# vr308/Generalised-Gaussian-Processes

Hardware: AMD Instinct MI355X
Metric: ELBO evals/sec (higher is better)
Workload: dtype f64

## Files before the change

generalised-gaussian-processes_amd/csrc/sgp_suffstats_fwd.hip:

```cpp
#include "sgp_common.hpp"
#include "sgp_stream.hpp"
#include "sgp_dense.hpp"
#include "sgp_composite.hpp"
#include "sgp_ctx.hpp"
#include <cstdlib>

namespace sgp {

static_assert(TIMING_SLOTS == CTX_TIMING_SLOTS, "timing slots");
size_t stream_kfu_budget() { return cur_ctx().kfu_budget; }

void timing_begin(int slot, hipStream_t st) {
  Ctx& c = cur_ctx();
  if (!c.timing) return;
  if (!c.ev_ready) {
    bool ok = true;
    for (int s = 0; s < TIMING_SLOTS; ++s)
      for (int k = 0; k < 2; ++k) ok = (hipEventCreate(&c.ev[s][k]) == hipSuccess) && ok;
    if (!ok) return;
    c.ev_ready = 1;
  }
  if (hipEventRecord(c.ev[slot][0], st) != hipSuccess) c.ev_used[slot] = 0;
}
void timing_end(int slot, hipStream_t st) {
// ... 236 lines not shown
        }
      };
#define SGP_DUMMY(cc, st) dummy(cc, st)
#else
#define SGP_DUMMY(cc, st)
#endif
      for (; c + 1 < c1; c += 2) {
        if (c + 2 < c1) fetch(c + 2, stA);
        mfma_chunk(0);
        SGP_DUMMY(c + 1, stB);
        stash(1, stB);
        __syncthreads();
        if (c + 3 < c1) fetch(c + 3, stB);
        mfma_chunk(1);
        if (c + 2 < c1) { SGP_DUMMY(c + 2, stA); }
        if (c + 2 < c1) stash(0, stA);
        __syncthreads();
      }
#ifdef SGP_AB_DIAG_DUMMY_ASM
      if (sink == 1.2345e300) out[0] = sink;
#endif
      if (c < c1) mfma_chunk(0);
    }
  
}

  if constexpr (BALANCED) {
    switch (wave) {
      case 0: diag_store<0>(acc, out, accumulate, l15, l4); break;
      case 1: diag_store<1>(acc, out, accumulate, l15, l4); break;
      case 2: diag_store<2>(acc, out, accumulate, l15, l4); break;
      default: diag_store<3>(acc, out, accumulate, l15, l4); break;
    }
    return;
  }
  {
#pragma unroll
    for (int u = 0; u < 4; ++u)
#pragma unroll
      for (int v = 0; v < VB; ++v)
#pragma unroll
        for (int r = 0; r < 4; ++r) {
          const int row = wi * 64 + u * 16 + l4 + 4 * r;
          const int col = wj * WCOLS + v * 16 + l15;
          double* dst = out + row * TILE + col;
          *dst = accumulate ? *dst + acc[u][v][r] : acc[u][v][r];
        }
  }
}

template <int NW, bool GLDS, bool SKIP>
__global__ __launch_bounds__(NW * 64, NW / 2) void syrk_tile_kernel(const double* __restrict__ Kfu, int Mp, int64_t nchunks,
                                                                    SplitMap smap, int ntiles, int accumulate,
                                                                    double* __restrict__ slab, int nsplit) {
  __shared__ double Ks[2][NB][KROW];
  const int id = blockIdx.x;
  const int xcd = id & 7;
  const int jj = id >> 3;
  const int full = (nsplit >> 3) * ntiles;
  int t, split;
  if (jj < full) {
    t = jj % ntiles;
    split = (jj / ntiles) * 8 + xcd;
  } else {
    const int rem = (nsplit & 7) * ntiles, per = (rem + 7) >> 3;
    const int u = xcd * per + (jj - full);
    if (jj - full >= per || u >= rem) return;
    t = u % ntiles;
    split = (nsplit & ~7) + u / ntiles;
  }
  int ti = (int)((sqrt(8.0 * t + 1.0) - 1.0) * 0.5);
  while ((ti + 1) * (ti + 2) / 2 <= t) ++ti;
  while (ti * (ti + 1) / 2 > t) --ti;
  const int tj = t - ti * (ti + 1) / 2;
  int64_t c0, c1;
  split_range(smap, split, nchunks, c0, c1);
  double* out = slab + ((size_t)split * ntiles + t) * (TILE * TILE);
  if (ti == tj)
    syrk_tile<true, NW, GLDS, SKIP>(Ks, Kfu, Mp, c0, c1, ti * TILE, tj * TILE, accumulate, out);
  else
    syrk_tile<false, NW, GLDS, SKIP>(Ks, Kfu, Mp, c0, c1, ti * TILE, tj * TILE, accumulate, out);
}

__global__ __launch_bounds__(256) void reduce_phi_kernel(const double* __restrict__ slab, int nsplit, int ntiles,
                                                         int M, double scale, double* __restrict__ Phi) {
  __shared__ double tile[32][33];
  const int t = blockIdx.x;
  int bi = (int)((sqrt(8.0 * t + 1.0) - 1.0) * 0.5);
  while ((bi + 1) * (bi + 2) / 2 <= t) ++bi;
  while (bi * (bi + 1) / 2 > t) --bi;
  const int bj = t - bi * (bi + 1) / 2;
  const int tx = threadIdx.x & 31, ty = threadIdx.x >> 5;
  const int Ti = (bi * 32) / TILE, Tj = (bj * 32) / TILE;
  const int tileidx = Ti * (Ti + 1) / 2 + Tj;
  const double* base = slab + (size_t)tileidx * (TILE * TILE);
  const size_t sstride = (size_t)ntiles * (TILE * TILE);
#pragma unroll
  for (int k = 0; k < 4; ++k) {
    const int lr = ty + 8 * k;
    const int gi = bi * 32 + lr, gj = bj * 32 + tx;
    double s = 0.0;
    if (gi >= gj) {
      const size_t off = (size_t)(gi - Ti * TILE) * TILE + (gj - Tj * TILE);
#pragma unroll 8
      for (int sp = 0; sp < nsplit; ++sp) s += base[sp * sstride + off];
    }
    tile[lr][tx] = s * scale;
  }
  __syncthreads();
#pragma unroll
  for (int k = 0; k < 4; ++k) {
    const int lr = ty + 8 * k;
    const int gi = bi * 32 + lr, gj = bj * 32 + tx;
    if (gi < M && gj < M && gi >= gj) Phi[(size_t)gi * M + gj] = tile[lr][tx];
    const int mi = bj * 32 + lr, mj = bi * 32 + tx;
    if (mi < M && mj < M && mj > mi) Phi[(size_t)mi * M + mj] = tile[tx][lr];
  }
}

__global__ __launch_bounds__(256) void bpart_stage1_kernel(const double* __restrict__ bpart, int64_t nrb, int Mp, int G,
                                                           double* __restrict__ tmp) {
  __shared__ double part[4][64];
  const int col = blockIdx.x * 64 + (threadIdx.x & 63), w = threadIdx.x >> 6, g = blockIdx.y;
  double s = 0.0;
  for (int64_t rb = g + (int64_t)w * G; rb < nrb; rb += 4 * (int64_t)G) s += bpart[rb * Mp + col];
  part[w][threadIdx.x & 63] = s;
  __syncthreads();
  if (w == 0) {
    const int l = threadIdx.x;
    tmp[(size_t)g * Mp + col] = (part[0][l] + part[1][l]) + (part[2][l] + part[3][l]);
  }
}

__global__ __launch_bounds__(256) void finalize_stats_kernel(const double* __restrict__ btmp, int G, int Mp, int M,
                                                             const double* __restrict__ yypart, int nyy, double sf2,
                                                             double kappa_val, double* __restrict__ b,
                                                             double* __restrict__ yy, double* __restrict__ kappa) {
  const int m = blockIdx.x * 256 + threadIdx.x;
  if (m < M) {
    double s = 0.0;
#pragma unroll 8
    for (int g = 0; g < G; ++g) s += btmp[(size_t)g * Mp + m];
    b[m] = s * sf2;
  }
  if (blockIdx.x == 0) {
    __shared__ double red[4];
    double s = 0.0;
    for (int i = threadIdx.x; i < nyy; i += 256) s += yypart[i];
    s = block_sum256(s, red);
    if (threadIdx.x == 0) {
      *yy = s;
      *kappa = kappa_val;
    }
  }
}

template <int DP, int ROWS>
static void launch_assemble_rows(int kid, dim3 grid, hipStream_t st, const double* Xs, const double* ys, const double* Zs,
                                 int64_t row0, int64_t N, int M, int Mp, double* Kfu, double* bpart) {
  switch (kid) {
    case SGP_KERNEL_RBF: kfu_assemble_kernel<DP, SGP_KERNEL_RBF, ROWS><<<grid, 256, 0, st>>>(Xs, ys, Zs, row0, N, M, Mp, Kfu, bpart); break;
    case SGP_KERNEL_MATERN32: kfu_assemble_kernel<DP, SGP_KERNEL_MATERN32, ROWS><<<grid, 256, 0, st>>>(Xs, ys, Zs, row0, N, M, Mp, Kfu, bpart); break;
    default: kfu_assemble_kernel<DP, SGP_KERNEL_MATERN52, ROWS><<<grid, 256, 0, st>>>(Xs, ys, Zs, row0, N, M, Mp, Kfu, bpart); break;
  }
}
template <int DP>
static void launch_assemble(int kid, int sub, dim3 grid, hipStream_t st, const double* Xs, const double* ys, const double* Zs,
                            int64_t row0, int64_t N, int M, int Mp, double* Kfu, double* bpart) {
  if (sub == 16) launch_assemble_rows<DP, ASM_ROWS / 16>(kid, grid, st, Xs, ys, Zs, row0, N, M, Mp, Kfu, bpart);
  else if (sub == 8) launch_assemble_rows<DP, ASM_ROWS / 8>(kid, grid, st, Xs, ys, Zs, row0, N, M, Mp, Kfu, bpart);
  else if (sub == 4) launch_assemble_rows<DP, ASM_ROWS / 4>(kid, grid, st, Xs, ys, Zs, row0, N, M, Mp, Kfu, bpart);
  else launch_assemble_rows<DP, ASM_ROWS>(kid, grid, st, Xs, ys, Zs, row0, N, M, Mp, Kfu, bpart);
}

void stream_assemble(const StreamPlan& p, int kid, const double* Xs, const double* ys, const double* Zs, int64_t row0,
                     int64_t rows, int64_t N, int M, double* Kfu, double* bpart, hipStream_t st) {
  dim3 grid((unsigned)(rows / ASM_ROWS * p.asm_sub), (p.Mp + 255) / 256);
  switch (p.DP) {
    case 2: launch_assemble<2>(kid, p.asm_sub, grid, st, Xs, ys, Zs, row0, N, M, p.Mp, Kfu, bpart); break;
    case 4: launch_assemble<4>(kid, p.asm_sub, grid, st, Xs, ys, Zs, row0, N, M, p.Mp, Kfu, bpart); break;
    case 8: launch_assemble<8>(kid, p.asm_sub, grid, st, Xs, ys, Zs, row0, N, M, p.Mp, Kfu, bpart); break;
    case 16: launch_assemble<16>(kid, p.asm_sub, grid, st, Xs, ys, Zs, row0, N, M, p.Mp, Kfu, bpart); break;
    case 24: launch_assemble<24>(kid, p.asm_sub, grid, st, Xs, ys, Zs, row0, N, M, p.Mp, Kfu, bpart); break;
    default: launch_assemble<32>(kid, p.asm_sub, grid, st, Xs, ys, Zs, row0, N, M, p.Mp, Kfu, bpart); break;
  }
}

void stream_prologue(const StreamPlan& p, const KernArgs& ka, const double* X, int64_t ldx, const double* y,
                     const double* Z, int64_t ldz, int64_t N, int M, double* Xs, double* ys, double* Zs, double* yypart,
                     hipStream_t st, const PadSymJob& pad) {
  int gx = 0;
  if (N > 0) {
    const int64_t tot = p.Npad * p.DP;
    gx = (int)((tot + 255) / 256 < 4096 ? (tot + 255) / 256 : 4096);
  }
  const int gz = (p.Mp * p.DP + 255) / 256;
  int gp = 0;
  if (pad.P) {
    const int64_t blocks = ((int64_t)p.Mp * p.Mp + 255) / 256;
// ... 390 lines not shown
  if (Kfu_out) p.sc_rows = p.Npad;
  FwdWs w = carve_fwd(ws, p, Kfu_out == nullptr, qrows);
  if (!ws || ws_bytes < w.bytes) return SGP_ERR_WORKSPACE;
  hipStream_t st = (hipStream_t)stream;

  KernArgs ka;
  for (int j = 0; j < SGP_MAX_DIM; ++j) ka.inv_ls[j] = j < d ? inv_ls[j] : 0.0;
  ka.sf2 = sf2;
  ka.d = d;

  stream_prologue(p, ka, X, ldx, y, Z, ldz, N, M, w.Xs, w.ys, w.Zs, w.yypart, st);
  double* Kfu = Kfu_out ? Kfu_out : w.Kfu;
  const int grid = p.ntiles * p.nsplit;
  if (p.Npad == 0) {
    syrk_tile_kernel<4, false, false><<<grid, 256, 0, st>>>(Kfu, p.Mp, 0, SplitMap{{0, 0, 0, 0}, 1}, p.ntiles, 0, w.slab, p.nsplit);
  }
  auto contract = [&](const double* K, int64_t nchunks, const SplitMap& smap, int nsplit, int accum, double* slab) {
    launch_syrk(cx, K, p.Mp, nchunks, smap, p.ntiles, nsplit, accum, slab, st);
  };
  int nslabs = p.nsplit;
  int head_ns = 0;
  int64_t head_chunks = 0;
  const bool use_i8 = i8_rule(cx.contraction, p.Npad, p.Mp);
  cx.contraction_used = use_i8 ? 1 : 0;
  if (!use_i8) gate = nullptr;
  if (p.Npad > 0 && !use_i8) head_block(p, p.Npad / NB, &head_ns, &head_chunks);
  if (use_i8) {
    const int ns = i8_nsplit(qrows, p.Mp);
    for (int64_t r0 = 0; r0 < p.Npad; r0 += qrows) {
      const int64_t rows = (p.Npad - r0) < qrows ? (p.Npad - r0) : qrows;
      timing_begin(TIMING_ASSEMBLE, st);
      i8_assemble(p, kernel_id, w.Xs, w.ys, w.Zs, r0, rows, N, M, w.Q, Kfu_out ? Kfu_out + (size_t)r0 * p.Mp : nullptr, w.bpart, st);
      timing_end(TIMING_ASSEMBLE, st);
      if (gate && hipStreamWaitEvent(st, gate, 0) != hipSuccess) return SGP_ERR_LAUNCH;
      gate = nullptr;
      timing_begin(TIMING_SYRK, st);
      if (i8_contract(w.Q, p.Mp, rows, ns, r0 > 0 ? 1 : 0, w.slab, st) != SGP_OK) return SGP_ERR_LAUNCH;
      timing_end(TIMING_SYRK, st);
      cx.syrk_timed_rows = rows;
    }
    nslabs = ns;
  } else if (head_ns > 0) {
    const int64_t hrows = head_chunks * NB, trows = p.Npad - hrows, tchunks = trows / NB;
    const bool side = cx.asm_overlap == 1 && side_stream_ready(cx);
    double* head_slab = w.slab + (size_t)p.nsplit * p.ntiles * TILE * TILE;
    const int hcps = (int)((head_chunks + head_ns - 1) / head_ns);
    const int tcps = (int)((tchunks + p.nsplit - 1) / p.nsplit);
    const SplitMap hmap{{0, 0, 0, 0}, hcps < 1 ? 1 : hcps};
    const SplitMap tmap{{p.taper[0], p.taper[1], p.taper[2], p.taper[3]}, tcps < 1 ? 1 : tcps};
    timing_begin(TIMING_ASSEMBLE, st);
    stream_assemble(p, kernel_id, w.Xs, w.ys, w.Zs, 0, hrows, N, M, Kfu, w.bpart, st);
    bool forked = false;
    if (side && hipEventRecord(cx.ev_fork, st) == hipSuccess && hipStreamWaitEvent(cx.side, cx.ev_fork, 0) == hipSuccess) {
      stream_assemble(p, kernel_id, w.Xs, w.ys, w.Zs, hrows, trows, N, M, Kfu + (size_t)hrows * p.Mp, w.bpart, cx.side);
      forked = hipEventRecord(cx.ev_join, cx.side) == hipSuccess;
      if (!forked) (void)hipStreamSynchronize(cx.side);
    } else {
      stream_assemble(p, kernel_id, w.Xs, w.ys, w.Zs, hrows, trows, N, M, Kfu + (size_t)hrows * p.Mp, w.bpart, st);
    }
    timing_end(TIMING_ASSEMBLE, st);
    contract(Kfu, head_chunks, hmap, head_ns, 0, head_slab);
    if (forked && hipStreamWaitEvent(st, cx.ev_join, 0) != hipSuccess) (void)hipStreamSynchronize(cx.side);
    timing_begin(TIMING_SYRK, st);
    contract(Kfu + (size_t)hrows * p.Mp, tchunks, tmap, p.nsplit, 0, w.slab);
    timing_end(TIMING_SYRK, st);
    cx.syrk_timed_rows = trows;
    nslabs = p.nsplit + head_ns;
  } else {
    for (int64_t r0 = 0; r0 < p.Npad; r0 += p.sc_rows) {
      const int64_t rows = (p.Npad - r0) < p.sc_rows ? (p.Npad - r0) : p.sc_rows;
      timing_begin(TIMING_ASSEMBLE, st);
      stream_assemble(p, kernel_id, w.Xs, w.ys, w.Zs, r0, rows, N, M, Kfu, w.bpart, st);
      timing_end(TIMING_ASSEMBLE, st);
      const int64_t nchunks = rows / NB;
      const int cps = (int)((nchunks + p.nsplit - 1) / p.nsplit);
      const SplitMap smap{{p.taper[0], p.taper[1], p.taper[2], p.taper[3]}, cps < 1 ? 1 : cps};
      timing_begin(TIMING_SYRK, st);
      contract(Kfu, nchunks, smap, p.nsplit, r0 > 0 ? 1 : 0, w.slab);
      timing_end(TIMING_SYRK, st);
      cx.syrk_timed_rows = rows;
    }
  }
  const int nb32 = p.Mp / 32;
  reduce_phi_kernel<<<nb32 * (nb32 + 1) / 2, 256, 0, st>>>(w.slab, nslabs, p.ntiles, M, sf2 * sf2, Phi);
  bpart_stage1_kernel<<<dim3(p.Mp / 64, BRED_G), 256, 0, st>>>(w.bpart, p.Npad / ASM_ROWS * (use_i8 ? 1 : p.asm_sub), p.Mp, BRED_G, w.btmp);
  finalize_stats_kernel<<<(M + 255) / 256, 256, 0, st>>>(w.btmp, BRED_G, p.Mp, M, w.yypart, 256, sf2,
                                                         sf2 * (double)N, b, yy, kappa);
  return check_launch();
}

extern "C" size_t sgp_suffstats_whitened_rows_workspace_bytes(int64_t N, int M, int d, int caller_owns_t) {
  if (N < 0 || M <= 0 || d <= 0 || d > SGP_MAX_DIM || M > SGP_MAX_INDUCING) return 0;
  StreamPlan p = make_stream_plan(N, M, d);
  if (caller_owns_t) p.sc_rows = p.Npad;
  return carve_wh_rows(nullptr, p, caller_owns_t != 0).bytes;
}
extern "C" int sgp_suffstats_fwd_whitened_rows(const double* X, int64_t ldx, const double* y, const double* Z, int64_t ldz,
                                               const double* inv_ls, double sf2, int64_t N, int M, int d, int kernel_id,
                                               const double* kuu_linv, double* W, double* u, double* yy, double* kappa, double* T_out,
                                               void* ws, size_t ws_bytes, sgp_stream_t stream) {
  Ctx& cx = cur_ctx();
  if (!Z || !inv_ls || !kuu_linv || !W || !u || !yy || !kappa || N < 0 || M <= 0 || d <= 0 || ldz < d) return SGP_ERR_ARG;
  if (N > 0 && (!X || !y || ldx < d)) return SGP_ERR_ARG;
  if (kernel_id < 0 || kernel_id >= SGP_KERNEL_COMPOSITE) return SGP_ERR_ARG;
  if (d > SGP_MAX_DIM || M > SGP_MAX_INDUCING) return SGP_ERR_DIM;
  StreamPlan p = make_stream_plan(N, M, d);
  if (T_out) p.sc_rows = p.Npad;
  WhRowsWs w = carve_wh_rows(ws, p, T_out != nullptr);
  if (!ws || ws_bytes < w.bytes) return SGP_ERR_WORKSPACE;
  hipStream_t st = (hipStream_t)stream;
  KernArgs ka;
  for (int j = 0; j < SGP_MAX_DIM; ++j) ka.inv_ls[j] = j < d ? inv_ls[j] : 0.0;
  ka.sf2 = sf2;
  ka.d = d;
  stream_prologue(p, ka, X, ldx, y, Z, ldz, N, M, w.f.Xs, w.f.ys, w.f.Zs, w.f.yypart, st);
  transpose_square(kuu_linv, p.Mp, w.R, st);
  if (p.Npad == 0)
    syrk_tile_kernel<4, false, false><<<p.ntiles * p.nsplit, 256, 0, st>>>(w.f.Kfu, p.Mp, 0, SplitMap{{0, 0, 0, 0}, 1}, p.ntiles, 0, w.f.slab,
                                                                           p.nsplit);
  for (int64_t r0 = 0; r0 < p.Npad; r0 += p.sc_rows) {
    const int64_t rows = (p.Npad - r0) < p.sc_rows ? (p.Npad - r0) : p.sc_rows;
    double* T = T_out ? T_out + (size_t)r0 * p.Mp : w.T;
    timing_begin(TIMING_ASSEMBLE, st);
    stream_assemble(p, kernel_id, w.f.Xs, w.f.ys, w.f.Zs, r0, rows, N, M, w.f.Kfu, w.f.bpart, st);
    timing_end(TIMING_ASSEMBLE, st);
    GemmDesc g;
    g.A = w.f.Kfu; g.lda = p.Mp; g.B = w.R; g.ldb = p.Mp; g.C = T; g.ldc = p.Mp;
    g.m = (int)rows; g.n = p.Mp; g.k = p.Mp; g.khi_mask = 2;
    gemm(g, st);
    tpart_kernel<<<dim3((unsigned)(rows / ASM_ROWS), (p.Mp + 255) / 256), 256, 0, st>>>(T, w.f.ys, r0, p.Mp, w.f.bpart);
    const int64_t nchunks = rows / NB;
    const int cps = (int)((nchunks + p.nsplit - 1) / p.nsplit);
    const SplitMap smap{{p.taper[0], p.taper[1], p.taper[2], p.taper[3]}, cps < 1 ? 1 : cps};
    timing_begin(TIMING_SYRK, st);
    launch_syrk(cx, T, p.Mp, nchunks, smap, p.ntiles, p.nsplit, r0 > 0 ? 1 : 0, w.f.slab, st);
    timing_end(TIMING_SYRK, st);
    cx.syrk_timed_rows = rows;
  }
  const int nb32 = p.Mp / 32;
  reduce_phi_kernel<<<nb32 * (nb32 + 1) / 2, 256, 0, st>>>(w.f.slab, p.nsplit, p.ntiles, M, sf2 * sf2, W);
  bpart_stage1_kernel<<<dim3(p.Mp / 64, BRED_G), 256, 0, st>>>(w.f.bpart, p.Npad / ASM_ROWS, p.Mp, BRED_G, w.f.btmp);
  finalize_stats_kernel<<<(M + 255) / 256, 256, 0, st>>>(w.f.btmp, BRED_G, p.Mp, M, w.f.yypart, 256, sf2, sf2 * (double)N, u, yy, kappa);
  return check_launch();
}


extern "C" size_t sgp_suffstats_extended_workspace_bytes(int64_t N, int M, int d) {
  if (N < 0 || M <= 0 || d <= 0 || d > SGP_MAX_DIM || M > SGP_MAX_INDUCING) return 0;
  StreamPlan p = make_stream_plan(N, M, d);
  return carve_ext(nullptr, p, p.sc_rows).bytes;
}
extern "C" int sgp_suffstats_fwd_extended(const double* X, int64_t ldx, const double* y, const double* Z, int64_t ldz,
                                          const double* inv_ls, double sf2, int64_t N, int M, int d, int kernel_id,
                                          const double* kuu_linv, int level, double* W, double* u, double* yy, double* kappa,
                                          double* Kfu_out, void* ws, size_t ws_bytes, sgp_stream_t stream) {
  return sgp_suffstats_fwd_extended_ex(X, ldx, y, Z, ldz, inv_ls, sf2, N, M, d, kernel_id, kuu_linv, level, W, u, yy, kappa, Kfu_out,
                                       nullptr, ws, ws_bytes, stream);
}
extern "C" int sgp_suffstats_fwd_extended_ex(const double* X, int64_t ldx, const double* y, const double* Z, int64_t ldz,
                                             const double* inv_ls, double sf2, int64_t N, int M, int d, int kernel_id,
                                             const double* kuu_linv, int level, double* W, double* u, double* yy, double* kappa,
                                             double* Kfu_out, double* phi_diag, void* ws, size_t ws_bytes, sgp_stream_t stream) {
  return sgp_suffstats_fwd_extended_f16(X, ldx, y, Z, ldz, inv_ls, sf2, N, M, d, kernel_id, kuu_linv, level, W, u, yy, kappa, Kfu_out, nullptr,
                                        phi_diag, ws, ws_bytes, stream);
}
extern "C" int sgp_suffstats_fwd_extended_f16(const double* X, int64_t ldx, const double* y, const double* Z, int64_t ldz,
                                              const double* inv_ls, double sf2, int64_t N, int M, int d, int kernel_id,
                                              const double* kuu_linv, int level, double* W, double* u, double* yy, double* kappa,
                                              double* Kfu_out, uint16_t* Kfu_f16_out, double* phi_diag, void* ws, size_t ws_bytes,
                                              sgp_stream_t stream) {
  if (Kfu_f16_out && !Kfu_out) return SGP_ERR_ARG;
  if (!Z || !inv_ls || !kuu_linv || !W || !u || !yy || !kappa || N < 0 || M <= 0 || d <= 0 || ldz < d) return SGP_ERR_ARG;
  if (N > 0 && (!X || !y || ldx < d)) return SGP_ERR_ARG;
  if (kernel_id < 0 || kernel_id >= SGP_KERNEL_COMPOSITE || level < 1 || level > 2) return SGP_ERR_ARG;
  if (d > SGP_MAX_DIM || M > SGP_MAX_INDUCING) return SGP_ERR_DIM;
  StreamPlan p = make_stream_plan(N, M, d);
  const int64_t qrows = p.sc_rows;
  ExtWs w = carve_ext(ws, p, qrows);
  if (!ws || ws_bytes < w.bytes) return SGP_ERR_WORKSPACE;
  hipStream_t st = (hipStream_t)stream;
  KernArgs ka;
  for (int j = 0; j < SGP_MAX_DIM; ++j) ka.inv_ls[j] = j < d ? inv_ls[j] : 0.0;
  ka.sf2 = sf2;
  ka.d = d;
  stream_prologue(p, ka, X, ldx, y, Z, ldz, N, M, w.Xs, w.ys, w.Zs, w.yypart, st);
  const int ns = i8_nsplit(qrows > 0 ? qrows : 1, p.Mp);
  const size_t nslab = (size_t)ns * p.ntiles * TILE * TILE;
  if (p.Npad == 0) {
    fill_zero(w.slab, nslab, st);
    fill_zero(w.slab_lo, nslab, st);
  }
  for (int64_t r0 = 0; r0 < p.Npad; r0 += qrows) {
    const int64_t rows = (p.Npad - r0) < qrows ? (p.Npad - r0) : qrows;
    timing_begin(TIMING_ASSEMBLE, st);
    i8_assemble(p, kernel_id, w.Xs, w.ys, w.Zs, r0, rows, N, M, w.Q, Kfu_out ? Kfu_out + (size_t)r0 * p.Mp : nullptr, w.bpart, st,
                Kfu_f16_out ? Kfu_f16_out + (size_t)r0 * p.Mp : nullptr);
    timing_end(TIMING_ASSEMBLE, st);
    timing_begin(TIMING_SYRK, st);
    if (i8_contract(w.Q, p.Mp, rows, ns, r0 > 0 ? 1 : 0, w.slab, st, w.slab_lo, level) != SGP_OK) return SGP_ERR_LAUNCH;
    timing_end(TIMING_SYRK, st);
  }
  const int nb32 = p.Mp / 32;
  reduce_phi_dd_kernel<<<nb32 * (nb32 + 1) / 2, 256, 0, st>>>(w.slab, w.slab_lo, ns, p.ntiles, p.Mp, w.Ph, w.Pl);
  dd_launch(w.Ph, w.Pl, kuu_linv, p.Mp, w.Yh, w.Yl, 1, st, 2, 0);
  dd_launch(w.Yh, w.Yl, kuu_linv, p.Mp, w.Wh, w.Wl, 0, st, 2, 1);
  ext_w_out_kernel<<<1024, 256, 0, st>>>(w.Wh, w.Wl, M, p.Mp, sf2 * sf2, W);
  if (phi_diag) ext_phi_diag_kernel<<<(M + 255) / 256, 256, 0, st>>>(w.Ph, M, p.Mp, sf2 * sf2, phi_diag);
  fill_zero(w.bpad, p.Mp, st);
  bpart_stage1_kernel<<<dim3(p.Mp / 64, BRED_G), 256, 0, st>>>(w.bpart, p.Npad / ASM_ROWS, p.Mp, BRED_G, w.btmp);
  finalize_stats_kernel<<<(M + 255) / 256, 256, 0, st>>>(w.btmp, BRED_G, p.Mp, M, w.yypart, 256, sf2, sf2 * (double)N, w.bpad, yy, kappa);
  gemv(kuu_linv, p.Mp, p.Mp, false, w.bpad, w.upad, st);
  crop_copy(w.upad, 1, u, 1, M, 1, st);
  return check_launch();
}
```

generalised-gaussian-processes_amd/csrc/sgp_suffstats_i8.hip:

```cpp
#include <atomic>
#include "sgp_common.hpp"
#include "sgp_stream.hpp"
#include "sgp_ctx.hpp"
#include <cstdlib>
#include <type_traits>

namespace sgp {

typedef int i4v __attribute__((ext_vector_type(4)));
typedef int i16v __attribute__((ext_vector_type(16)));

constexpr int I8_NP = 7;
constexpr int I8_TR = 128, I8_TC = 64;
constexpr int I8_SCOLS = I8_TR + I8_TC;
constexpr int I8_STAGE_BYTES = 2 * I8_NP * I8_SCOLS * 16;
constexpr int I8_NSTAGE = 3;
constexpr int I8_PIECES = 2 * I8_NP * 3;
constexpr int I8_PPW = (I8_PIECES + 7) / 8;
constexpr int I8_LDS_BYTES = I8_NSTAGE * I8_STAGE_BYTES;

template <int DP, int KID, bool WK>
__global__ __launch_bounds__(256) void kfu_digits_kernel(const double* __restrict__ Xs, const double* __restrict__ ys,
                                                         const double* __restrict__ Zs, int64_t row0, int64_t N, int M, int Mp,
                                                         uint8_t* __restrict__ Q, double* __restrict__ Kfu, uint16_t* __restrict__ Kh,
// ... 9 lines not shown
    ysh[threadIdx.x] = ys[row0 + rbase + threadIdx.x];
    sgp_exp_tab_load(etab);
  }
  __syncthreads();
  const int m = blockIdx.y * 256 + threadIdx.x;
  if (m >= Mp) return;
  const double zmask = m < M ? 1.0 : 0.0;
  double zr[DP];
#pragma unroll
  for (int j = 0; j < DP; ++j) zr[j] = Zs[(size_t)m * DP + j];

  constexpr unsigned long long C = 0x0080808080808080ULL;
  double bacc = 0.0;
#ifdef SGP_AB_DIGITS_NO_INTERIOR
  const bool interior = false;
#else
  const bool interior = (row0 + rbase + ASM_ROWS <= N) && ((int)(blockIdx.y * 256 + 255) < M);
#endif
  auto run = [&](auto masked_tag) {
  constexpr bool MASKED = decltype(masked_tag)::value;
  for (int g = 0; g < ASM_ROWS / 16; ++g) {
    unsigned lo[16], hi[16];
#pragma unroll
    for (int e = 0; e < 16; ++e) {
      const int i = g * 16 + e;
      const int64_t n = row0 + rbase + i;
      double r2 = 0.0;
#pragma unroll
      for (int j = 0; j < DP; ++j) {
        const double df = xs[i][j] - zr[j];
        r2 = fma(df, df, r2);
      }
      double kv = kprofile_tab<KID>(r2, etab);
      if constexpr (MASKED) kv *= (n < N ? zmask : 0.0);
      bacc = fma(kv, ysh[i], bacc);
      if constexpr (WK) {
        __builtin_nontemporal_store(kv, &Kfu[(rbase + i) * Mp + m]);
        if (Kh) {
          float kf = (float)kv;
          asm volatile("" : "+v"(kf));
          Kh[(rbase + i) * Mp + m] = __builtin_bit_cast(uint16_t, (_Float16)kf);
        }
      }
      const double th = fma(kv, 0x1p22, 0x1p52);
      const double hf = th - 0x1p52;
      const double tl = fma(-hf, 0x1p32, kv * 0x1p54) + 0x1.8p52;
      const unsigned long long tb = (unsigned long long)__double_as_longlong(tl);
      const unsigned q_hi = (unsigned)__double_as_longlong(th) - ((unsigned)(tb >> 32) & 1u);
      const unsigned long long q = ((unsigned long long)q_hi << 32) | (unsigned)tb;
      const unsigned long long qq = (q + C) ^ C;
      lo[e] = (unsigned)qq;
      hi[e] = (unsigned)(qq >> 32);
    }
    const size_t rb = (size_t)(rbase / 16 + g);
    i4v plane[8];
#pragma unroll
    for (int j = 0; j < 4; ++j) {
#pragma unroll
      for (int h = 0; h < 2; ++h) {
        const unsigned* s4 = (h ? hi : lo) + 4 * j;
        const unsigned u0 = __builtin_amdgcn_perm(s4[1], s4[0], 0x05010400u), u1 = __builtin_amdgcn_perm(s4[1], s4[0], 0x07030602u);
        const unsigned v0 = __builtin_amdgcn_perm(s4[3], s4[2], 0x05010400u), v1 = __builtin_amdgcn_perm(s4[3], s4[2], 0x07030602u);
        plane[4 * h + 0][j] = (int)__builtin_amdgcn_perm(v0, u0, 0x05040100u);
        plane[4 * h + 1][j] = (int)__builtin_amdgcn_perm(v0, u0, 0x07060302u);
        plane[4 * h + 2][j] = (int)__builtin_amdgcn_perm(v1, u1, 0x05040100u);
        if (h == 0) plane[3][j] = (int)__builtin_amdgcn_perm(v1, u1, 0x07060302u);
      }
    }
#pragma unroll
    for (int p = 0; p < I8_NP; ++p)
      __builtin_nontemporal_store(plane[p], reinterpret_cast<i4v*>(Q + ((rb * I8_NP + p) * Mp + m) * 16));
  }
  };
  if (interior) run(std::false_type{}); else run(std::true_type{});
  bpart[((row0 + rbase) / ASM_ROWS) * Mp + m] = bacc;
}

constexpr int I8_PSPLIT = 5;
#ifdef SGP_AB_I8_PAIRS34
constexpr int I8_MINSUM_DEFAULT = 5;
#else
constexpr int I8_MINSUM_DEFAULT = 6;
#endif
static_assert(2 * I8_PPW - 1 <= I8_PSPLIT * (I8_PSPLIT + 1) / 2, "every DMA piece must find its MFMA in the first half");

template <bool ACT, int I8_MINSUM, bool DD>
__device__ __forceinline__ void i8_tile_loop(uint8_t* lds, const uint8_t* __restrict__ Q, int Mp, int64_t c0, int64_t c1, int I0,
                                             int J0, int accumulate, double* __restrict__ out, size_t lo_off, int wave, int lane, int prio) {
  constexpr int I8_NG = 13 - I8_MINSUM;
  const int grp = wave >> 2, w4 = wave & 3;
  const int wi = (w4 >> 1) * 2 + grp, wj = w4 & 1;
  const int l32 = lane & 31, lh = lane >> 5;
  i16v acc[I8_NG];
#pragma unroll
  for (int g = 0; g < I8_NG; ++g)
#pragma unroll
    for (int r = 0; r < 16; ++r) acc[g][r] = 0;

  unsigned goff[I8_PPW];
  int soff[I8_PPW];
#pragma unroll
  for (int k = 0; k < I8_PPW; ++k) {
    int e = wave + 8 * k;
    if (e >= I8_PIECES) e -= I8_PIECES;
    const int rbl = e / (I8_NP * 3), rem = e % (I8_NP * 3), p = rem / 3, cg = rem % 3;
    const int col = cg < 2 ? I0 + cg * 64 : J0;
    goff[k] = (unsigned)(((rbl * I8_NP + p) * Mp + col + lane) * 16);
    soff[k] = __builtin_amdgcn_readfirstlane(((rbl * I8_NP + p) * I8_SCOLS + cg * 64) * 16);
  }
  const size_t gstride = (size_t)2 * I8_NP * Mp * 16;
  auto dma_piece = [&](const uint8_t* gbase, int sbase, int k) {
    __builtin_amdgcn_global_load_lds((const __attribute__((address_space(1))) void*)(gbase + goff[k]),
                                     (__attribute__((address_space(3))) void*)(lds + sbase + soff[k]), 16, 0, 0);
  };
  const int64_t nst = c1 - c0;
  auto wait_stage = [&](int64_t sE) {
    if (sE + 1 >= nst)
      __builtin_amdgcn_s_waitcnt(0 | (7 << 4) | (15 << 8));
    else
      __builtin_amdgcn_s_waitcnt((I8_PPW & 15) | ((I8_PPW >> 4) << 14) | (7 << 4) | (15 << 8));
  };
  auto bar = [&]() {
    __builtin_amdgcn_s_barrier();
    asm volatile("" ::: "memory");
  };
  i4v b[I8_NP], a[I8_NP];
  auto reads = [&](int64_t sidx) {
    if (ACT) {
      const uint8_t* sb = lds + (int)(sidx % I8_NSTAGE) * I8_STAGE_BYTES + lh * (I8_NP * I8_SCOLS * 16);
#pragma unroll
      for (int p = 0; p < I8_NP; ++p) {
        b[I8_NP - 1 - p] = *reinterpret_cast<const i4v*>(sb + ((I8_NP - 1 - p) * I8_SCOLS + I8_TR + wj * 32 + l32) * 16);
        a[p] = *reinterpret_cast<const i4v*>(sb + (p * I8_SCOLS + wi * 32 + l32) * 16);
      }
    }
    __builtin_amdgcn_sched_barrier(0);
  };
  auto half = [&](int p0, int p1, bool dma_on, int64_t sE) {
    if (prio) { if (dma_on) __builtin_amdgcn_s_setprio(1); else __builtin_amdgcn_s_setprio(0); }
    const bool pre = dma_on && sE + 2 < nst;
    const uint8_t* gnext = Q + (size_t)(c0 + sE + 2) * gstride;
    const int snext = (int)((sE + 2) % I8_NSTAGE) * I8_STAGE_BYTES;
    int issued = 0, kpiece = 0;
#pragma unroll
    for (int p = p0; p < p1; ++p)
#pragma unroll
      for (int r = (I8_MINSUM - p > 0 ? I8_MINSUM - p : 0); r < I8_NP; ++r) {
        if (ACT) acc[p + r - I8_MINSUM] = __builtin_amdgcn_mfma_i32_32x32x32_i8(a[p], b[r], acc[p + r - I8_MINSUM], 0, 0, 0);
        ++issued;
        if (dma_on && (issued & 1) && kpiece < I8_PPW) {
          __builtin_amdgcn_sched_barrier(0);
          if (pre) dma_piece(gnext, snext, kpiece);
          __builtin_amdgcn_sched_barrier(0);
          ++kpiece;
        }
      }
  };
  if (nst > 0) {
#pragma unroll
    for (int k = 0; k < I8_PPW; ++k) dma_piece(Q + (size_t)c0 * gstride, 0, k);
    if (nst > 1) {
#pragma unroll
      for (int k = 0; k < I8_PPW; ++k) dma_piece(Q + (size_t)(c0 + 1) * gstride, I8_STAGE_BYTES, k);
    }
    if (grp == 0) {
      for (int64_t sidx = 0; sidx < nst; ++sidx) {
        wait_stage(sidx);
        bar();
        reads(sidx);
        half(0, I8_PSPLIT, true, sidx);
        bar();
        half(I8_PSPLIT, I8_NP, false, sidx);
      }
      wait_stage(nst);
      bar();
    } else {
      wait_stage(0);
      bar();
      for (int64_t sidx = 0; sidx < nst; ++sidx) {
        bar();
        reads(sidx);
        half(0, I8_PSPLIT, true, sidx);
        __builtin_amdgcn_s_waitcnt(15 | (3 << 14) | (7 << 4) | (0 << 8));
        wait_stage(sidx + 1);
        bar();
        half(I8_PSPLIT, I8_NP, false, sidx + 1);
      }
    }
  }
  if (ACT) {
#pragma unroll
    for (int r = 0; r < 16; ++r) {
      const int row = wi * 32 + (r >> 2) * 8 + lh * 4 + (r & 3);
      double* dst = out + row * TILE + wj * 32 + l32;
      if constexpr (DD) {
#pragma clang fp contract(off)
        double hi = 0.0, lo = 0.0;
        if (accumulate) { hi = dst[0]; lo = dst[lo_off]; }
#pragma unroll
        for (int g = 0; g < I8_NG; ++g) {
          const double t = (double)acc[g][r] * __builtin_ldexp(1.0, 8 * (g + I8_MINSUM) - 108);
          const double sum = hi + t;
          const double z = sum - hi;
          lo += (hi - (sum - z)) + (t - z);
          hi = sum;
        }
        const double sum = hi + lo;
        dst[lo_off] = lo - (sum - hi);
        dst[0] = sum;
      } else {
        double v = 0.0;
#pragma unroll
        for (int g = 0; g < I8_NG; ++g) v = fma((double)acc[g][r], __builtin_ldexp(1.0, 8 * (g + I8_MINSUM) - 108), v);
        *dst = accumulate ? *dst + v : v;
      }
    }
  }
}

template <int MINSUM, bool DD>
__global__ __launch_bounds__(512, 1) void i8_syrk_tile_kernel(const uint8_t* __restrict__ Q, int Mp, int64_t nsteps, int nsplit,
                                                              int ntiles, int ntiles128, int accumulate, double* __restrict__ slab,
                                                              size_t lo_off, int prio) {
  extern __shared__ __attribute__((aligned(16))) uint8_t i8_lds[];
  const int id = blockIdx.x;
  const int xcd = id & 7, jj = id >> 3;
  const int t = jj % ntiles, split = (jj / ntiles) * 8 + xcd;
  if (split >= nsplit) return;
  int ti = (int)((sqrtf(4.0f * t + 1.0f) - 1.0f) * 0.5f);
  while ((ti + 1) * (ti + 2) <= t) ++ti;
  while (ti * (ti + 1) > t) --ti;
  const int tj = t - ti * (ti + 1);
  const int I0 = ti * I8_TR, J0 = tj * I8_TC;
  int64_t c0, c1;
  i8_split_steps(nsteps, nsplit, split, c0, c1);
  const int lane = threadIdx.x & 63;
  const int wave = __builtin_amdgcn_readfirstlane(threadIdx.x >> 6);
  double* out = slab + ((size_t)split * ntiles128 + (ti * (ti + 1) / 2 + (tj >> 1))) * (TILE * TILE) + (tj & 1) * I8_TC;
  const int grp = wave >> 2, w4 = wave & 3;
  const int wi = (w4 >> 1) * 2 + grp, wj = w4 & 1;
  if (J0 + 32 * wj <= I0 + 32 * wi + 31)
    i8_tile_loop<true, MINSUM, DD>(i8_lds, Q, Mp, c0, c1, I0, J0, accumulate, out, lo_off, wave, lane, prio);
  else
    i8_tile_loop<false, MINSUM, DD>(i8_lds, Q, Mp, c0, c1, I0, J0, accumulate, out, lo_off, wave, lane, prio);
}

template <int DP, bool WK>
static void launch_digits(int kid, dim3 grid, hipStream_t st, const double* Xs, const double* ys, const double* Zs, int64_t row0,
                          int64_t N, int M, int Mp, uint8_t* Q, double* Kfu, uint16_t* Kh, double* bpart) {
  switch (kid) {
    case SGP_KERNEL_RBF: kfu_digits_kernel<DP, SGP_KERNEL_RBF, WK><<<grid, 256, 0, st>>>(Xs, ys, Zs, row0, N, M, Mp, Q, Kfu, Kh, bpart); break;
    case SGP_KERNEL_MATERN32: kfu_digits_kernel<DP, SGP_KERNEL_MATERN32, WK><<<grid, 256, 0, st>>>(Xs, ys, Zs, row0, N, M, Mp, Q, Kfu, Kh, bpart); break;
    default: kfu_digits_kernel<DP, SGP_KERNEL_MATERN52, WK><<<grid, 256, 0, st>>>(Xs, ys, Zs, row0, N, M, Mp, Q, Kfu, Kh, bpart); break;
  }
}
template <bool WK>
static void launch_digits_dp(int DP, int kid, dim3 grid, hipStream_t st, const double* Xs, const double* ys, const double* Zs,
                             int64_t row0, int64_t N, int M, int Mp, uint8_t* Q, double* Kfu, uint16_t* Kh, double* bpart) {
  switch (DP) {
    case 2: launch_digits<2, WK>(kid, grid, st, Xs, ys, Zs, row0, N, M, Mp, Q, Kfu, Kh, bpart); break;
    case 4: launch_digits<4, WK>(kid, grid, st, Xs, ys, Zs, row0, N, M, Mp, Q, Kfu, Kh, bpart); break;
    case 8: launch_digits<8, WK>(kid, grid, st, Xs, ys, Zs, row0, N, M, Mp, Q, Kfu, Kh, bpart); break;
    case 16: launch_digits<16, WK>(kid, grid, st, Xs, ys, Zs, row0, N, M, Mp, Q, Kfu, Kh, bpart); break;
    case 24: launch_digits<24, WK>(kid, grid, st, Xs, ys, Zs, row0, N, M, Mp, Q, Kfu, Kh, bpart); break;
    default: launch_digits<32, WK>(kid, grid, st, Xs, ys, Zs, row0, N, M, Mp, Q, Kfu, Kh, bpart); break;
  }
}

void i8_assemble(const StreamPlan& p, int kid, const double* Xs, const double* ys, const double* Zs, int64_t row0, int64_t rows,
                 int64_t N, int M, uint8_t* Q, double* Kfu, double* bpart, hipStream_t st, uint16_t* Kh) {
  dim3 grid((unsigned)(rows / ASM_ROWS), (p.Mp + 255) / 256);
  if (Kfu)
    launch_digits_dp<true>(p.DP, kid, grid, st, Xs, ys, Zs, row0, N, M, p.Mp, Q, Kfu, Kh, bpart);
  else
    launch_digits_dp<false>(p.DP, kid, grid, st, Xs, ys, Zs, row0, N, M, p.Mp, Q, nullptr, nullptr, bpart);
}

int i8_contract(const uint8_t* Q, int Mp, int64_t rows, int nsplit, int accumulate, double* slab, hipStream_t st, double* slab_lo, int level) {
  Ctx& cx = cur_ctx();
  static std::atomic<bool> attr_done[64];
  int dev = 0;
  if (hipGetDevice(&dev) != hipSuccess || dev < 0) return SGP_ERR_LAUNCH;
  if (dev >= 64 || !attr_done[dev].load(std::memory_order_acquire)) {
    if (hipFuncSetAttribute((const void*)i8_syrk_tile_kernel<I8_MINSUM_DEFAULT, false>, hipFuncAttributeMaxDynamicSharedMemorySize,
                            I8_LDS_BYTES) != hipSuccess ||
        hipFuncSetAttribute((const void*)i8_syrk_tile_kernel<5, true>, hipFuncAttributeMaxDynamicSharedMemorySize, I8_LDS_BYTES) !=
            hipSuccess ||
        hipFuncSetAttribute((const void*)i8_syrk_tile_kernel<4, true>, hipFuncAttributeMaxDynamicSharedMemorySize, I8_LDS_BYTES) !=
            hipSuccess)
      return SGP_ERR_LAUNCH;
    if (dev < 64) attr_done[dev].store(true, std::memory_order_release);
  }
  const int nrt = Mp / I8_TR, ntiles = nrt * (nrt + 1), ntiles128 = nrt * (nrt + 1) / 2;
  const int prio = cx.i8_prio;
  if (slab_lo && level >= 2)
    i8_syrk_tile_kernel<4, true><<<nsplit * ntiles, 512, I8_LDS_BYTES, st>>>(Q, Mp, rows / 32, nsplit, ntiles, ntiles128, accumulate, slab,
                                                                             (size_t)(slab_lo - slab), prio);
  else if (slab_lo)
    i8_syrk_tile_kernel<5, true><<<nsplit * ntiles, 512, I8_LDS_BYTES, st>>>(Q, Mp, rows / 32, nsplit, ntiles, ntiles128, accumulate, slab,
                                                                             (size_t)(slab_lo - slab), prio);
  else
    i8_syrk_tile_kernel<I8_MINSUM_DEFAULT, false><<<nsplit * ntiles, 512, I8_LDS_BYTES, st>>>(Q, Mp, rows / 32, nsplit, ntiles, ntiles128,
                                                                                               accumulate, slab, 0, prio);
  return SGP_OK;
}

}
```

Before: 70.17.

## Exploit symmetry on diagonal i8 SYRK blocks, trim duplicate DMA, split reduce_phi

Waves on diagonal 32x32 blocks now issue only the upper-triangular digit-pair MFMAs and fold the mirrored products back in through an LDS transpose. This roughly halves the diagonal MFMA work. When the J block lies inside the same 128-column panel as I, the redundant column-group DMA is skipped and the vmcnt waits are adjusted to match the per-wave piece count. reduce_phi is split into four row parts per tile with wider, independent loads to raise parallelism, at the cost of more extra registers, LDS traffic and code complexity.

```diff
diff --git a/generalised-gaussian-processes_amd/csrc/sgp_suffstats_fwd.hip b/generalised-gaussian-processes_amd/csrc/sgp_suffstats_fwd.hip
--- a/generalised-gaussian-processes_amd/csrc/sgp_suffstats_fwd.hip
+++ b/generalised-gaussian-processes_amd/csrc/sgp_suffstats_fwd.hip
@@ -342,10 +342,16 @@
     syrk_tile<false, NW, GLDS, SKIP>(Ks, Kfu, Mp, c0, c1, ti * TILE, tj * TILE, accumulate, out);
 }
 
+#ifdef SGP_AB_REDUCE_PHI_CHAIN
+constexpr int REDUCE_PHI_SPLIT = 1;
+#else
+constexpr int REDUCE_PHI_SPLIT = 4;
+#endif
 __global__ __launch_bounds__(256) void reduce_phi_kernel(const double* __restrict__ slab, int nsplit, int ntiles,
                                                          int M, double scale, double* __restrict__ Phi) {
-  __shared__ double tile[32][33];
-  const int t = blockIdx.x;
+  constexpr int ROWS = 32 / REDUCE_PHI_SPLIT, NK = ROWS / 8;
+  __shared__ double tile[ROWS][33];
+  const int t = blockIdx.x / REDUCE_PHI_SPLIT, part = blockIdx.x % REDUCE_PHI_SPLIT;
   int bi = (int)((sqrt(8.0 * t + 1.0) - 1.0) * 0.5);
   while ((bi + 1) * (bi + 2) / 2 <= t) ++bi;
   while (bi * (bi + 1) / 2 > t) --bi;
@@ -356,25 +362,39 @@
   const double* base = slab + (size_t)tileidx * (TILE * TILE);
   const size_t sstride = (size_t)ntiles * (TILE * TILE);
 #pragma unroll
-  for (int k = 0; k < 4; ++k) {
+  for (int k = 0; k < NK; ++k) {
     const int lr = ty + 8 * k;
-    const int gi = bi * 32 + lr, gj = bj * 32 + tx;
+    const int gi = bi * 32 + part * ROWS + lr, gj = bj * 32 + tx;
     double s = 0.0;
     if (gi >= gj) {
       const size_t off = (size_t)(gi - Ti * TILE) * TILE + (gj - Tj * TILE);
+#ifdef SGP_AB_REDUCE_PHI_CHAIN
 #pragma unroll 8
       for (int sp = 0; sp < nsplit; ++sp) s += base[sp * sstride + off];
+#else
+      for (int sp0 = 0; sp0 < nsplit; sp0 += 32) {
+        double v[32];
+#pragma unroll
+        for (int u = 0; u < 32; ++u) v[u] = sp0 + u < nsplit ? base[(size_t)(sp0 + u) * sstride + off] : 0.0;
+#pragma unroll
+        for (int u = 0; u < 32; ++u)
+          if (sp0 + u < nsplit) s += v[u];
+      }
+#endif
     }
     tile[lr][tx] = s * scale;
   }
   __syncthreads();
 #pragma unroll
-  for (int k = 0; k < 4; ++k) {
+  for (int k = 0; k < NK; ++k) {
     const int lr = ty + 8 * k;
-    const int gi = bi * 32 + lr, gj = bj * 32 + tx;
+    const int gi = bi * 32 + part * ROWS + lr, gj = bj * 32 + tx;
     if (gi < M && gj < M && gi >= gj) Phi[(size_t)gi * M + gj] = tile[lr][tx];
-    const int mi = bj * 32 + lr, mj = bi * 32 + tx;
-    if (mi < M && mj < M && mj > mi) Phi[(size_t)mi * M + mj] = tile[tx][lr];
+  }
+  for (int e = threadIdx.x; e < 32 * ROWS; e += 256) {
+    const int c = e / ROWS, lr = e % ROWS;
+    const int mi = bj * 32 + c, mj = bi * 32 + part * ROWS + lr;
+    if (mi < M && mj < M && mj > mi) Phi[(size_t)mi * M + mj] = tile[lr][c];
   }
 }
 
@@ -931,7 +951,7 @@
     }
   }
   const int nb32 = p.Mp / 32;
-  reduce_phi_kernel<<<nb32 * (nb32 + 1) / 2, 256, 0, st>>>(w.slab, nslabs, p.ntiles, M, sf2 * sf2, Phi);
+  reduce_phi_kernel<<<REDUCE_PHI_SPLIT * (nb32 * (nb32 + 1) / 2), 256, 0, st>>>(w.slab, nslabs, p.ntiles, M, sf2 * sf2, Phi);
   bpart_stage1_kernel<<<dim3(p.Mp / 64, BRED_G), 256, 0, st>>>(w.bpart, p.Npad / ASM_ROWS * (use_i8 ? 1 : p.asm_sub), p.Mp, BRED_G, w.btmp);
   finalize_stats_kernel<<<(M + 255) / 256, 256, 0, st>>>(w.btmp, BRED_G, p.Mp, M, w.yypart, 256, sf2,
                                                          sf2 * (double)N, b, yy, kappa);
@@ -987,7 +1007,7 @@
     cx.syrk_timed_rows = rows;
   }
   const int nb32 = p.Mp / 32;
-  reduce_phi_kernel<<<nb32 * (nb32 + 1) / 2, 256, 0, st>>>(w.f.slab, p.nsplit, p.ntiles, M, sf2 * sf2, W);
+  reduce_phi_kernel<<<REDUCE_PHI_SPLIT * (nb32 * (nb32 + 1) / 2), 256, 0, st>>>(w.f.slab, p.nsplit, p.ntiles, M, sf2 * sf2, W);
   bpart_stage1_kernel<<<dim3(p.Mp / 64, BRED_G), 256, 0, st>>>(w.f.bpart, p.Npad / ASM_ROWS, p.Mp, BRED_G, w.f.btmp);
   finalize_stats_kernel<<<(M + 255) / 256, 256, 0, st>>>(w.f.btmp, BRED_G, p.Mp, M, w.f.yypart, 256, sf2, sf2 * (double)N, u, yy, kappa);
   return check_launch();
diff --git a/generalised-gaussian-processes_amd/csrc/sgp_suffstats_i8.hip b/generalised-gaussian-processes_amd/csrc/sgp_suffstats_i8.hip
--- a/generalised-gaussian-processes_amd/csrc/sgp_suffstats_i8.hip
+++ b/generalised-gaussian-processes_amd/csrc/sgp_suffstats_i8.hip
@@ -115,28 +115,53 @@
 #else
 constexpr int I8_MINSUM_DEFAULT = 6;
 #endif
-static_assert(2 * I8_PPW - 1 <= I8_PSPLIT * (I8_PSPLIT + 1) / 2, "every DMA piece must find its MFMA in the first half");
-
-template <bool ACT, int I8_MINSUM, bool DD>
+enum { I8_ROLE_IDLE = 0, I8_ROLE_ACT = 1, I8_ROLE_DIAG = 2 };
+constexpr int i8_first_half_mfmas(int minsum, bool diag) {
+  int n = 0;
+  for (int p = 0; p < I8_PSPLIT; ++p)
+    for (int r = (minsum - p > 0 ? minsum - p : 0); r < I8_NP; ++r) n += (!diag || r >= p) ? 1 : 0;
+  return n;
+}
+static_assert(2 * I8_PPW - 1 <= i8_first_half_mfmas(6, false) && 2 * I8_PPW - 1 <= i8_first_half_mfmas(6, true) &&
+              2 * I8_PPW - 1 <= i8_first_half_mfmas(5, true) && 2 * I8_PPW - 1 <= i8_first_half_mfmas(4, true),
+              "every DMA piece must find its MFMA in the first half, in every role");
+constexpr int i8_vmcnt(int n) { return (n & 15) | ((n >> 4) << 14) | (7 << 4) | (15 << 8); }
+
+template <int ROLE, int I8_MINSUM, bool DD>
 __device__ __forceinline__ void i8_tile_loop(uint8_t* lds, const uint8_t* __restrict__ Q, int Mp, int64_t c0, int64_t c1, int I0,
                                              int J0, int accumulate, double* __restrict__ out, size_t lo_off, int wave, int lane, int prio) {
+  constexpr bool ACT = ROLE != I8_ROLE_IDLE, DIAG = ROLE == I8_ROLE_DIAG;
   constexpr int I8_NG = 13 - I8_MINSUM;
+  constexpr int NACC = DIAG ? I8_NG + (I8_NG - 1) / 2 : I8_NG;
   const int grp = wave >> 2, w4 = wave & 3;
   const int wi = (w4 >> 1) * 2 + grp, wj = w4 & 1;
   const int l32 = lane & 31, lh = lane >> 5;
-  i16v acc[I8_NG];
-#pragma unroll
-  for (int g = 0; g < I8_NG; ++g)
+  i16v acc[NACC];
+#pragma unroll
+  for (int g = 0; g < NACC; ++g)
 #pragma unroll
     for (int r = 0; r < 16; ++r) acc[g][r] = 0;
 
+#ifdef SGP_AB_I8_DMA_REPEAT
+  constexpr bool jin = false;
+  constexpr int npw = I8_PPW;
+#else
+  const bool jin = (J0 >> 7) == (I0 >> 7);
+  const int npw = __builtin_amdgcn_readfirstlane(((jin ? 2 * I8_NP * 2 : I8_PIECES) - wave + 7) >> 3);
+#endif
   unsigned goff[I8_PPW];
   int soff[I8_PPW];
 #pragma unroll
   for (int k = 0; k < I8_PPW; ++k) {
     int e = wave + 8 * k;
-    if (e >= I8_PIECES) e -= I8_PIECES;
-    const int rbl = e / (I8_NP * 3), rem = e % (I8_NP * 3), p = rem / 3, cg = rem % 3;
+    int rbl, p, cg;
+    if (jin) {
+      if (e >= 2 * I8_NP * 2) e = wave;
+      rbl = e / (I8_NP * 2), p = (e % (I8_NP * 2)) / 2, cg = e % 2;
+    } else {
+      if (e >= I8_PIECES) e -= I8_PIECES;
+      rbl = e / (I8_NP * 3), p = (e % (I8_NP * 3)) / 3, cg = (e % (I8_NP * 3)) % 3;
+    }
     const int col = cg < 2 ? I0 + cg * 64 : J0;
     goff[k] = (unsigned)(((rbl * I8_NP + p) * Mp + col + lane) * 16);
     soff[k] = __builtin_amdgcn_readfirstlane(((rbl * I8_NP + p) * I8_SCOLS + cg * 64) * 16);
@@ -149,21 +174,34 @@
   const int64_t nst = c1 - c0;
   auto wait_stage = [&](int64_t sE) {
     if (sE + 1 >= nst)
-      __builtin_amdgcn_s_waitcnt(0 | (7 << 4) | (15 << 8));
+      __builtin_amdgcn_s_waitcnt(i8_vmcnt(0));
+    else if (npw == 6)
+      __builtin_amdgcn_s_waitcnt(i8_vmcnt(6));
+    else if (npw == 5)
+      __builtin_amdgcn_s_waitcnt(i8_vmcnt(5));
+    else if (npw == 4)
+      __builtin_amdgcn_s_waitcnt(i8_vmcnt(4));
     else
-      __builtin_amdgcn_s_waitcnt((I8_PPW & 15) | ((I8_PPW >> 4) << 14) | (7 << 4) | (15 << 8));
+      __builtin_amdgcn_s_waitcnt(i8_vmcnt(3));
   };
   auto bar = [&]() {
     __builtin_amdgcn_s_barrier();
     asm volatile("" ::: "memory");
   };
   i4v b[I8_NP], a[I8_NP];
+  const int bcol = jin ? J0 - I0 + wj * 32 : I8_TR + wj * 32;
   auto reads = [&](int64_t sidx) {
-    if (ACT) {
-      const uint8_t* sb = lds + (int)(sidx % I8_NSTAGE) * I8_STAGE_BYTES + lh * (I8_NP * I8_SCOLS * 16);
+    const uint8_t* sb = lds + (int)(sidx % I8_NSTAGE) * I8_STAGE_BYTES + lh * (I8_NP * I8_SCOLS * 16);
+    if (DIAG) {
+#pragma unroll
+      for (int k = 0; k < I8_NP; ++k) {
+        const int p = (k & 1) ? I8_NP - 1 - (k >> 1) : (k >> 1);
+        a[p] = *reinterpret_cast<const i4v*>(sb + (p * I8_SCOLS + wi * 32 + l32) * 16);
+      }
+    } else if (ACT) {
 #pragma unroll
       for (int p = 0; p < I8_NP; ++p) {
-        b[I8_NP - 1 - p] = *reinterpret_cast<const i4v*>(sb + ((I8_NP - 1 - p) * I8_SCOLS + I8_TR + wj * 32 + l32) * 16);
+        b[I8_NP - 1 - p] = *reinterpret_cast<const i4v*>(sb + ((I8_NP - 1 - p) * I8_SCOLS + bcol + l32) * 16);
         a[p] = *reinterpret_cast<const i4v*>(sb + (p * I8_SCOLS + wi * 32 + l32) * 16);
       }
     }
@@ -171,7 +209,7 @@
   };
   auto half = [&](int p0, int p1, bool dma_on, int64_t sE) {
     if (prio) { if (dma_on) __builtin_amdgcn_s_setprio(1); else __builtin_amdgcn_s_setprio(0); }
-    const bool pre = dma_on && sE + 2 < nst;
+    const int npre = dma_on && sE + 2 < nst ? npw : 0;
     const uint8_t* gnext = Q + (size_t)(c0 + sE + 2) * gstride;
     const int snext = (int)((sE + 2) % I8_NSTAGE) * I8_STAGE_BYTES;
     int issued = 0, kpiece = 0;
@@ -179,11 +217,14 @@
     for (int p = p0; p < p1; ++p)
 #pragma unroll
       for (int r = (I8_MINSUM - p > 0 ? I8_MINSUM - p : 0); r < I8_NP; ++r) {
-        if (ACT) acc[p + r - I8_MINSUM] = __builtin_amdgcn_mfma_i32_32x32x32_i8(a[p], b[r], acc[p + r - I8_MINSUM], 0, 0, 0);
+        if (DIAG && r < p) continue;
+        const int g = p + r - I8_MINSUM;
+        const int slot = DIAG && p == r && g < I8_NG - 1 ? I8_NG + (g >> 1) : g;
+        if (ACT) acc[slot] = __builtin_amdgcn_mfma_i32_32x32x32_i8(a[p], DIAG ? a[r] : b[r], acc[slot], 0, 0, 0);
         ++issued;
         if (dma_on && (issued & 1) && kpiece < I8_PPW) {
           __builtin_amdgcn_sched_barrier(0);
-          if (pre) dma_piece(gnext, snext, kpiece);
+          if (kpiece < npre) dma_piece(gnext, snext, kpiece);
           __builtin_amdgcn_sched_barrier(0);
           ++kpiece;
         }
@@ -191,10 +232,12 @@
   };
   if (nst > 0) {
 #pragma unroll
-    for (int k = 0; k < I8_PPW; ++k) dma_piece(Q + (size_t)c0 * gstride, 0, k);
+    for (int k = 0; k < I8_PPW; ++k)
+      if (k < npw) dma_piece(Q + (size_t)c0 * gstride, 0, k);
     if (nst > 1) {
 #pragma unroll
-      for (int k = 0; k < I8_PPW; ++k) dma_piece(Q + (size_t)(c0 + 1) * gstride, I8_STAGE_BYTES, k);
+      for (int k = 0; k < I8_PPW; ++k)
+        if (k < npw) dma_piece(Q + (size_t)(c0 + 1) * gstride, I8_STAGE_BYTES, k);
     }
     if (grp == 0) {
       for (int64_t sidx = 0; sidx < nst; ++sidx) {
@@ -219,6 +262,27 @@
         bar();
         half(I8_PSPLIT, I8_NP, false, sidx + 1);
       }
+    }
+  }
+  if constexpr (DIAG) {
+    int* xt = reinterpret_cast<int*>(lds) + wave * (32 * 33);
+#pragma unroll
+    for (int g = 0; g < I8_NG - 1; ++g) {
+#pragma unroll
+      for (int r = 0; r < 16; ++r) xt[((r >> 2) * 8 + lh * 4 + (r & 3)) * 33 + l32] = acc[g][r];
+      __builtin_amdgcn_fence(__ATOMIC_RELEASE, "wavefront");
+      __builtin_amdgcn_wave_barrier();
+      __builtin_amdgcn_fence(__ATOMIC_ACQUIRE, "wavefront");
+#pragma unroll
+      for (int r = 0; r < 16; ++r) {
+        int v = acc[g][r] + xt[l32 * 33 + (r >> 2) * 8 + lh * 4 + (r & 3)];
+        if (((g + I8_MINSUM) & 1) == 0) v += acc[I8_NG + (g >> 1)][r];
+        acc[g][r] = v;
+      }
+      asm volatile("" : "+v"(acc[g]));
+      __builtin_amdgcn_fence(__ATOMIC_RELEASE, "wavefront");
+      __builtin_amdgcn_wave_barrier();
+      __builtin_amdgcn_fence(__ATOMIC_ACQUIRE, "wavefront");
     }
   }
   if (ACT) {
@@ -272,10 +336,15 @@
   double* out = slab + ((size_t)split * ntiles128 + (ti * (ti + 1) / 2 + (tj >> 1))) * (TILE * TILE) + (tj & 1) * I8_TC;
   const int grp = wave >> 2, w4 = wave & 3;
   const int wi = (w4 >> 1) * 2 + grp, wj = w4 & 1;
+#ifndef SGP_AB_I8_DIAG_FULL
+  if (J0 + 32 * wj == I0 + 32 * wi)
+    i8_tile_loop<I8_ROLE_DIAG, MINSUM, DD>(i8_lds, Q, Mp, c0, c1, I0, J0, accumulate, out, lo_off, wave, lane, prio);
+  else
+#endif
   if (J0 + 32 * wj <= I0 + 32 * wi + 31)
-    i8_tile_loop<true, MINSUM, DD>(i8_lds, Q, Mp, c0, c1, I0, J0, accumulate, out, lo_off, wave, lane, prio);
+    i8_tile_loop<I8_ROLE_ACT, MINSUM, DD>(i8_lds, Q, Mp, c0, c1, I0, J0, accumulate, out, lo_off, wave, lane, prio);
   else
-    i8_tile_loop<false, MINSUM, DD>(i8_lds, Q, Mp, c0, c1, I0, J0, accumulate, out, lo_off, wave, lane, prio);
+    i8_tile_loop<I8_ROLE_IDLE, MINSUM, DD>(i8_lds, Q, Mp, c0, c1, I0, J0, accumulate, out, lo_off, wave, lane, prio);
 }
 
 template <int DP, bool WK>
```

Result: slower. 67.47 (-3.8%).
